# cocowy1/Cost-Volume-Aggregation-in-Stereo-Matching-Revisited

Hardware: AMD Instinct MI355X
Metric: cost-volumes/sec (fwd+bwd) at 544x960 D=192 (higher is better)
Workload: dtype f32

## Files before the change

cost-volume-aggregation-in-stereo-matching-revisited_amd/csrc/pointwise.hip:

```cpp
#include "bn_math.h"
#include "../../include/dca_hip.h"

__global__ __launch_bounds__(256) void bn_stats_kernel(const float* __restrict__ x, double* __restrict__ part, int N,
                                                       int C, long S, int nchunk, long chunk_len, int vec) {
  const int c = blockIdx.x, ch = blockIdx.y, tid = threadIdx.x;
  const long s0 = ch * chunk_len, s1 = min(S, s0 + chunk_len);
  const float K = x[(long)c * S];
  if (ch == 0 && tid == 0) part[(long)C * nchunk * 2 + c] = (double)K;
  float s = 0.f, ss = 0.f;
  for (int n = 0; n < N; ++n) {
    const float* p = x + ((long)n * C + c) * S;
    if (vec) {
      for (long i = s0 + 4 * tid; i < s1; i += 1024) {
        float4 v = *(const float4*)(p + i);
        v.x -= K; v.y -= K; v.z -= K; v.w -= K;
        s += (v.x + v.y) + (v.z + v.w);
        ss += (v.x * v.x + v.y * v.y) + (v.z * v.z + v.w * v.w);
      }
    } else {
      for (long i = s0 + tid; i < s1; i += 256) {
        const float v = p[i] - K;
        s += v;
        ss += v * v;
      }
// ... 590 lines not shown
  }
}

__global__ __launch_bounds__(256) void avgpool3d_fwd_tiled_kernel(const float* __restrict__ x, float* __restrict__ y,
                                                                  int Di, int Hi, int Wi, int Do, int Ho, int Wo) {
  constexpr int TH = 8, TW = 32, FH = 2 * TH + 1, PW = 2 * TW + 2;
  __shared__ __attribute__((aligned(16))) float tile[3 * FH * PW];
  const int tid = threadIdx.x, ow0 = blockIdx.x * TW, oh0 = blockIdx.y * TH;
  const int od = blockIdx.z % Do;
  const long nc = blockIdx.z / Do;
  const long plane = (long)Di * Hi * Wi;
  const __amdgpu_buffer_rsrc_t xr = dca_rsrc(x + nc * plane, plane * 4);
  constexpr int NQ = 3 * FH * 16, KQ = (NQ + 255) / 256;
  float4 rq[KQ];
#pragma unroll
  for (int k = 0; k < KQ; ++k) {
    const int it = tid + 256 * k, q = it & 15, row = it >> 4, a = row / FH, b = row - a * FH;
    const int d = 2 * od - 1 + a, h = 2 * oh0 - 1 + b, w = 2 * ow0 + 4 * q;
    const int ok = (int)(it < NQ) & (int)((unsigned)d < (unsigned)Di) & (int)((unsigned)h < (unsigned)Hi) & (int)(w < Wi);
    rq[k] = dca_bload4(xr, ((d * Hi + h) * Wi + w) * 4, ok);
  }
  float redge = 0.f;
  {
    const int a = tid / FH, b = tid - a * FH;
    const int d = 2 * od - 1 + a, h = 2 * oh0 - 1 + b, w = 2 * ow0 - 1;
    const int ok = (int)(tid < 3 * FH) & (int)((unsigned)d < (unsigned)Di) & (int)((unsigned)h < (unsigned)Hi) &
                   (int)((unsigned)w < (unsigned)Wi);
    redge = dca_bload1(xr, ((d * Hi + h) * Wi + w) * 4, ok);
  }
#pragma unroll
  for (int k = 0; k < KQ; ++k) {
    const int it = tid + 256 * k;
    if (it < NQ) {
      float* p = tile + (it >> 4) * PW + 1 + 4 * (it & 15);
      p[0] = rq[k].x; p[1] = rq[k].y; p[2] = rq[k].z; p[3] = rq[k].w;
    }
  }
  if (tid < 3 * FH) tile[tid * PW] = redge;
  __syncthreads();
  const int hl = tid >> 5, wl = tid & 31, oh = oh0 + hl, ow = ow0 + wl;
  if (oh >= Ho || ow >= Wo) return;
  float s = 0.f;
#pragma unroll
  for (int kd = 0; kd < 3; ++kd)
#pragma unroll
    for (int kh = 0; kh < 3; ++kh) {
      const float* row = tile + (kd * FH + 2 * hl + kh) * PW + 2 * wl;
      const float2 lo = *(const float2*)row;
      s += lo.x;
      s += lo.y;
      s += row[2];
    }
  y[((nc * Do + od) * Ho + oh) * (long)Wo + ow] = s * (1.0f / 27.0f);
}

__global__ __launch_bounds__(256) void avgpool3d_bwd_vec_kernel(const float* __restrict__ gy, float* __restrict__ gx,
                                                                const float* __restrict__ res, const float* __restrict__ res2,
                                                                int Di, int Hi, int Wi, int Do, int Ho, int Wo) {
  const int BD = Di / 2 + 1, BH = Hi / 2 + 1;
  const int bd = (int)(blockIdx.x % BD);
  const long nc = blockIdx.x / BD;
  const long plane = (long)Do * Ho * Wo;
  const __amdgpu_buffer_rsrc_t gr = dca_rsrc(gy + nc * plane, plane * 4);
  const int WQ = Wi >> 2, HQ = BH * WQ, end = min(HQ, ((int)blockIdx.y + 1) * 1024);
  for (int i = blockIdx.y * 1024 + threadIdx.x; i < end; i += 256) {
    const int bh = i / WQ, t = i - bh * WQ, c0 = 2 * t;
    float g[2][2][3];
#pragma unroll
    for (int a = 0; a < 2; ++a)
#pragma unroll
      for (int b = 0; b < 2; ++b)
#pragma unroll
        for (int c = 0; c < 3; ++c) {
          const int od = bd - 1 + a, oh = bh - 1 + b, ow = c0 + c;
          const int ok = (int)((unsigned)od < (unsigned)Do) & (int)((unsigned)oh < (unsigned)Ho) & (int)(ow < Wo);
          g[a][b][c] = dca_bload1(gr, ((od * Ho + oh) * Wo + ow) * 4, ok);
        }
#pragma unroll
    for (int pd = 0; pd < 2; ++pd) {
      const int d = 2 * bd - 1 + pd;
      if ((unsigned)d >= (unsigned)Di) continue;
#pragma unroll
      for (int ph = 0; ph < 2; ++ph) {
        const int h = 2 * bh - 1 + ph;
        if ((unsigned)h >= (unsigned)Hi) continue;
        float o[4];
#pragma unroll
        for (int e = 0; e < 4; ++e) {
          float s = 0.f;
#pragma unroll
          for (int a = pd; a < 2; ++a)
#pragma unroll
            for (int b = ph; b < 2; ++b) {
              s += g[a][b][e >> 1];
              s += (e & 1) ? g[a][b][(e + 1) >> 1] : 0.f;
            }
          o[e] = s * (1.0f / 27.0f);
        }
        const long off = ((nc * Di + d) * Hi + h) * (long)Wi + 4 * t;
        if (res) {
          const float4 r = *(const float4*)(res + off);
          o[0] += r.x; o[1] += r.y; o[2] += r.z; o[3] += r.w;
        }
        if (res2) {
          const float4 r = *(const float4*)(res2 + off);
          o[0] += r.x; o[1] += r.y; o[2] += r.z; o[3] += r.w;
// ... 72 lines not shown
        if (wh == 0.f) continue;
        const float* row = p + ((long)od * Ho + oh) * Wo;
        float r = 0.f;
        for (int ow = ow0; ow <= ow1; ++ow) r += lin_w(ow, w, rs, Wi) * row[ow];
        acc += wd * wh * r;
      }
    }
    gx[idx] = acc;
  }
}

__global__ __launch_bounds__(256) void trilinear_up2_fwd_kernel(const float* __restrict__ x, float* __restrict__ y,
                                                                int Di, int Hi, int Wi) {
  const int mw = blockIdx.x * 64 + (threadIdx.x & 63), mh = blockIdx.y * 4 + (threadIdx.x >> 6);
  const int md = blockIdx.z % Di;
  const long nc = blockIdx.z / Di;
  if (mw >= Wi || mh >= Hi) return;
  const float* p = x + nc * Di * Hi * Wi;
  const int dm = max(md - 1, 0), dp = min(md + 1, Di - 1), hm = max(mh - 1, 0), hp = min(mh + 1, Hi - 1);
  const int wm = max(mw - 1, 0), wp = min(mw + 1, Wi - 1);
  float r0[3][3], r1[3][3];
  const int ds[3] = {dm, md, dp}, hs[3] = {hm, mh, hp};
#pragma unroll
  for (int a = 0; a < 3; ++a)
#pragma unroll
    for (int b = 0; b < 3; ++b) {
      const float* row = p + ((long)ds[a] * Hi + hs[b]) * Wi;
      const float xm = row[wm], x0 = row[mw], xp = row[wp];
      r0[a][b] = 0.25f * xm + 0.75f * x0;
      r1[a][b] = 0.75f * x0 + 0.25f * xp;
    }
  const int Ho = 2 * Hi, Wo = 2 * Wi;
  float* q = y + nc * (2L * Di) * Ho * Wo;
#pragma unroll
  for (int pd = 0; pd < 2; ++pd)
#pragma unroll
    for (int ph = 0; ph < 2; ++ph) {
      const int a0 = pd ? 1 : 0, a1 = pd ? 2 : 1, b0 = ph ? 1 : 0, b1 = ph ? 2 : 1;
      const float wa0 = pd ? 0.75f : 0.25f, wa1 = pd ? 0.25f : 0.75f, wb0 = ph ? 0.75f : 0.25f, wb1 = ph ? 0.25f : 0.75f;
      float2 o;
      o.x = wa0 * (wb0 * r0[a0][b0] + wb1 * r0[a0][b1]) + wa1 * (wb0 * r0[a1][b0] + wb1 * r0[a1][b1]);
      o.y = wa0 * (wb0 * r1[a0][b0] + wb1 * r1[a0][b1]) + wa1 * (wb0 * r1[a1][b0] + wb1 * r1[a1][b1]);
      *(float2*)(q + ((long)(2 * md + pd) * Ho + 2 * mh + ph) * Wo + 2 * mw) = o;
    }
}

__device__ __forceinline__ void up2_bwd_w(int i, int n, float w[4]) {
  w[0] = (i > 0) ? 0.25f : 0.f;
  w[1] = (i > 0) ? 0.75f : 1.0f;
  w[2] = (i < n - 1) ? 0.75f : 1.0f;
  w[3] = (i < n - 1) ? 0.25f : 0.f;
}

__global__ __launch_bounds__(256) void trilinear_up2_bwd_kernel(const float* __restrict__ gy, float* __restrict__ gx,
                                                                int Di, int Hi, int Wi) {
  const int w = blockIdx.x * 256 + threadIdx.x, h = blockIdx.y;
  const int d = blockIdx.z % Di;
  const long nc = blockIdx.z / Di;
  const int Ho = 2 * Hi, Wo = 2 * Wi;
  const long plane = (2L * Di) * Ho * Wo;
  const __amdgpu_buffer_rsrc_t gr = dca_rsrc(gy + nc * plane, plane * 4);
  const int wok = (int)(w < Wi);
  float wd[4], wh[4], ww[4];
  up2_bwd_w(d, Di, wd); up2_bwd_w(h, Hi, wh); up2_bwd_w(w, Wi, ww);
  float acc = 0.f;
#pragma unroll
  for (int a = 0; a < 4; ++a) {
    const int od = 2 * d - 1 + a;
#pragma unroll
    for (int b = 0; b < 4; ++b) {
      const int oh = 2 * h - 1 + b;
      const int ok = wok & (int)(wd[a] != 0.f) & (int)(wh[b] != 0.f);
      const int off = ((od * Ho + oh) * Wo + 2 * w) * 4;
      const float2 mid = dca_bload2(gr, off, ok);
      const float lo = dca_bload1(gr, off - 4, ok & (int)(ww[0] != 0.f));
      const float hi = dca_bload1(gr, off + 8, ok & (int)(ww[3] != 0.f));
      float r = ww[1] * mid.x + ww[2] * mid.y;
      r += ww[0] * lo;
      r += ww[3] * hi;
      acc += wd[a] * wh[b] * r;
    }
  }
  if (wok) gx[((nc * Di + d) * Hi + h) * Wi + w] = acc;
}

__global__ __launch_bounds__(256) void trilinear_up2_bwd_tiled_kernel(const float* __restrict__ gy, float* __restrict__ gx,
                                                                      int Di, int Hi, int Wi) {
  constexpr int TH = 8, TW = 32, FH = 2 * TH + 2, FW = 2 * TW + 2, PW = FW + 2;
  __shared__ __attribute__((aligned(16))) float tile[4 * FH * PW];
  const int tid = threadIdx.x, w0 = blockIdx.x * TW, h0 = blockIdx.y * TH;
  const int d = blockIdx.z % Di;
  const long nc = blockIdx.z / Di;
  const int Do = 2 * Di, Ho = 2 * Hi, Wo = 2 * Wi;
  const long plane = (long)Do * Ho * Wo;
  const __amdgpu_buffer_rsrc_t gr = dca_rsrc(gy + nc * plane, plane * 4);
  constexpr int NQ = 4 * FH * 16, KQ = (NQ + 255) / 256;
  float4 rq[KQ];
#pragma unroll
  for (int k = 0; k < KQ; ++k) {
    const int it = tid + 256 * k, q = it & 15, row = it >> 4, a = row / FH, b = row - a * FH;
    const int od = 2 * d - 1 + a, oh = 2 * h0 - 1 + b, ow = 2 * w0 + 4 * q;
    const int ok = (int)(it < NQ) & (int)((unsigned)od < (unsigned)Do) & (int)((unsigned)oh < (unsigned)Ho) &
                   (int)(ow < Wo);
    rq[k] = dca_bload4(gr, ((od * Ho + oh) * Wo + ow) * 4, ok);
  }
  float redge = 0.f;
  {
    const int side = tid & 1, row = tid >> 1, a = row / FH, b = row - a * FH;
    const int od = 2 * d - 1 + a, oh = 2 * h0 - 1 + b, ow = side ? 2 * w0 + 2 * TW : 2 * w0 - 1;
    const int ok = (int)(tid < 4 * FH * 2) & (int)((unsigned)od < (unsigned)Do) & (int)((unsigned)oh < (unsigned)Ho) &
                   (int)((unsigned)ow < (unsigned)Wo);
    redge = dca_bload1(gr, ((od * Ho + oh) * Wo + ow) * 4, ok);
  }
#pragma unroll
  for (int k = 0; k < KQ; ++k) {
    const int it = tid + 256 * k;
    if (it < NQ) {
      float* p = tile + (it >> 4) * PW + 1 + 4 * (it & 15);
      p[0] = rq[k].x; p[1] = rq[k].y; p[2] = rq[k].z; p[3] = rq[k].w;
    }
  }
  if (tid < 4 * FH * 2) tile[(tid >> 1) * PW + ((tid & 1) ? FW - 1 : 0)] = redge;
  __syncthreads();
  const int hl = tid >> 5, wl = tid & 31, h = h0 + hl, w = w0 + wl;
  if (h >= Hi || w >= Wi) return;
  float wd[4], wh[4], ww[4];
  up2_bwd_w(d, Di, wd); up2_bwd_w(h, Hi, wh); up2_bwd_w(w, Wi, ww);
  float acc = 0.f;
#pragma unroll
  for (int a = 0; a < 4; ++a)
#pragma unroll
    for (int b = 0; b < 4; ++b) {
      const float* row = tile + (a * FH + 2 * hl + b) * PW + 2 * wl;
      const float2 lo = *(const float2*)row, hi = *(const float2*)(row + 2);
      float r = ww[1] * lo.y + ww[2] * hi.x;
      r += ww[0] * lo.x;
      r += ww[3] * hi.y;
      acc += wd[a] * wh[b] * r;
    }
  gx[((nc * Di + d) * Hi + h) * Wi + w] = acc;
}

static int ew_grid(long total) {
  long g = (total + 255) / 256;
  return (int)(g < 8192 ? (g > 0 ? g : 1) : 8192);
}

static void chunking(long S, int C, int* nchunk, long* chunk_len) {
  long want = (2048 + C - 1) / C;
  if (want > 256) want = 256;
  long len = (S + want - 1) / want;
  len = ((len + 1023) / 1024) * 1024;
  *chunk_len = len;
  *nchunk = (int)((S + len - 1) / len);
}

extern "C" int dca_bn_num_chunks(int C, long S) {
  int n; long l;
  chunking(S, C, &n, &l);
  return n;
}
extern "C" int dca_bn_pack_chunks(int C, long S) {
  int n; long l;
  chunking(S, (C + 7) / 8, &n, &l);
  return n;
}

extern "C" int dca_bn_stats(const float* x, double* part, int N, int C, long S, hipStream_t stream) {
  DCA_REQUIRE(x && part && N > 0 && C > 0 && S > 0 && C <= 65535);
  int nchunk; long len;
  chunking(S, C, &nchunk, &len);
  const int vec = (S % 4 == 0) && (((uintptr_t)x & 15) == 0);
  hipLaunchKernelGGL(bn_stats_kernel, dim3(C, nchunk), dim3(256), 0, stream, x, part, N, C, S, nchunk, len, vec);
  return dca_launch_status();
}

extern "C" int dca_bn_finalize(const double* part, int nchunk, double count, const float* gamma, const float* beta,
                               float* running_mean, float* running_var, float momentum, float eps, int training,
                               float* stats, int* zexps, const unsigned* rpre_slots, int rpre_n,
                               const unsigned* rpost_slots, int rpost_n, int C, hipStream_t stream) {
  DCA_REQUIRE(stats && C > 0 && (training ? (part != nullptr && nchunk > 0) : (running_mean && running_var)));
  DCA_REQUIRE(zexps == nullptr || training);
  DCA_REQUIRE((rpre_slots == nullptr || (rpre_n > 0 && rpre_n <= DCA_AMAX_CSLOTS)) &&
              (rpost_slots == nullptr || (rpost_n > 0 && rpost_n <= DCA_AMAX_CSLOTS)));
  hipLaunchKernelGGL(bn_finalize_kernel, dim3(C), dim3(64), 0, stream, part, nchunk, count, gamma, beta,
                     running_mean, running_var, momentum, eps, training, stats, zexps, rpre_slots, rpre_n, rpost_slots,
                     rpost_n, C);
  return dca_launch_status();
}

extern "C" int dca_bn_finalize_centered(const double* part, int nchunk, const float* gamma, const float* beta,
                                        float* running_mean, float* running_var, float momentum, float eps, float* stats,
                                        int* zexps, const unsigned* rpre_slots, int rpre_n, const unsigned* rpost_slots,
// ... 107 lines not shown
  hipLaunchKernelGGL(bn_bwd_finalize_kernel, dim3(C), dim3(64), 0, stream, part, nchunk, count, dgb, C, stats, training,
                     (const unsigned*)nullptr, (const unsigned*)nullptr, 0, (int*)nullptr);
  hipLaunchKernelGGL(bn_bwd_finalize_kernel, dim3(C), dim3(64), 0, stream, (const double*)part_r, nchunk, count, dgb_r, C,
                     stats_r, training, (const unsigned*)nullptr, (const unsigned*)nullptr, 0, (int*)nullptr);
  hipLaunchKernelGGL(bn_bwd_apply_kernel, dim3(nchunk, C), dim3(256), 0, stream, dz, y, (const float*)nullptr, stats, dgb, dy,
                     g_out, N, C, S, len, slope, training, vec, dmax, y_r, stats_r);
  return dca_launch_status();
}

extern "C" int dca_bn_backward_reduce(const float* dz, const float* y, const float* stats, double* part, float* dgb, int N,
                                      int C, long S, float slope, int training, hipStream_t stream) {
  DCA_REQUIRE(dz && y && stats && part && dgb && N > 0 && C > 0 && S > 0 && C <= 65535);
  int nchunk; long len;
  chunking(S, C, &nchunk, &len);
  const int vec = (S % 4 == 0) && ((((uintptr_t)dz | (uintptr_t)y) & 15) == 0);
  hipLaunchKernelGGL(bn_bwd_reduce_kernel, dim3(C, nchunk), dim3(256), 0, stream, dz, y, (const float*)nullptr, stats, part,
                     N, C, S, nchunk, len, slope, vec, (unsigned*)nullptr, (const float*)nullptr, (const float*)nullptr,
                     (double*)nullptr);
  hipLaunchKernelGGL(bn_bwd_finalize_kernel, dim3(C), dim3(64), 0, stream, part, nchunk, (double)N * (double)S, dgb, C,
                     stats, training, (const unsigned*)nullptr, (const unsigned*)nullptr, 0, (int*)nullptr);
  return dca_launch_status();
}

void dca_internal_bn_chunking(long S, int C, int* nchunk, long* chunk_len) { chunking(S, C, nchunk, chunk_len); }

int dca_internal_bn_bwd_finalize(const double* part, int nchunk, double count, float* dgb, int C, const float* stats,
                                 int training, const unsigned* gmax, const unsigned* ymax, int ymax_slots, int* dyexps,
                                 hipStream_t stream) {
  hipLaunchKernelGGL(bn_bwd_finalize_kernel, dim3(C), dim3(64), 0, stream, part, nchunk, count, dgb, C, stats, training, gmax,
                     ymax, ymax_slots, dyexps);
  return dca_launch_status();
}

extern "C" int dca_bn_backward_pack(const float* dz, const float* y, const float* stats, double* part, float* dgb, void* dyp,
                                    int* dyexps, unsigned* gmax, const unsigned* ymax, int ymax_slots, int N, int C, long S,
                                    float slope, int training, hipStream_t stream) {
  DCA_REQUIRE(dz && y && stats && part && dgb && dyp && dyexps && gmax && N > 0 && C > 0 && C % 8 == 0 && S > 0 && C <= 65535);
  DCA_REQUIRE((ymax == nullptr || (ymax_slots > 0 && ymax_slots <= DCA_AMAX_CSLOTS)) && ((((uintptr_t)dyp) & 15) == 0));
  int nchunk; long len;
  chunking(S, C, &nchunk, &len);
  const uintptr_t al = (uintptr_t)dz | (uintptr_t)y;
  const int vec = (S % 4 == 0) && ((al & 15) == 0);
  hipLaunchKernelGGL(bn_bwd_reduce_kernel, dim3(C, nchunk), dim3(256), 0, stream, dz, y, (const float*)nullptr, stats, part,
                     N, C, S, nchunk, len, slope, vec, gmax, (const float*)nullptr, (const float*)nullptr, (double*)nullptr);
  hipLaunchKernelGGL(bn_bwd_finalize_kernel, dim3(C), dim3(64), 0, stream, part, nchunk, (double)N * (double)S, dgb, C,
                     stats, training, (const unsigned*)gmax, ymax, ymax_slots, dyexps);
  int pchunk; long plen;
  chunking(S, C / 8, &pchunk, &plen);
  hipLaunchKernelGGL(bn_bwd_apply_pack_kernel, dim3(pchunk, C / 8), dim3(256), 0, stream, dz, y, stats, dgb, dyexps,
                     (char*)dyp, N, C, S, plen, slope, training);
  return dca_launch_status();
}

extern "C" int dca_avgpool3d_fwd(const float* x, float* y, long NC, int Di, int Hi, int Wi, hipStream_t stream) {
  DCA_REQUIRE(x && y && NC > 0 && Di > 0 && Hi > 0 && Wi > 0);
  const int Do = (Di + 1) / 2, Ho = (Hi + 1) / 2, Wo = (Wi + 1) / 2;
  DCA_REQUIRE((long)Di * Hi * Wi * 4 < 0x7ffffff0L && NC * Do < 0x7fffffffL);
  if (Wi % 4 == 0 && (((uintptr_t)x) & 15) == 0 && NC * Do <= 65535 && cdiv(Ho, 8) <= 65535) {
    hipLaunchKernelGGL(avgpool3d_fwd_tiled_kernel, dim3(cdiv(Wo, 32), cdiv(Ho, 8), (unsigned)(NC * Do)), dim3(256), 0, stream,
                       x, y, Di, Hi, Wi, Do, Ho, Wo);
    return dca_launch_status();
  }
  hipLaunchKernelGGL(avgpool3d_fwd_kernel, dim3((unsigned)(NC * Do), cdiv((long)Ho * Wo, 1024)), dim3(256), 0, stream, x,
                     y, Di, Hi, Wi, Do, Ho, Wo);
  return dca_launch_status();
}

extern "C" int dca_avgpool3d_bwd(const float* gy, float* gx, const float* res, const float* res2, long NC, int Di, int Hi,
                                 int Wi, hipStream_t stream) {
  DCA_REQUIRE(gy && gx && NC > 0 && Di > 0 && Hi > 0 && Wi > 0 && (res || !res2));
  const int Do = (Di + 1) / 2, Ho = (Hi + 1) / 2, Wo = (Wi + 1) / 2;
  DCA_REQUIRE((long)Di * Hi * Wi * 4 < 0x7ffffff0L && NC * Di < 0x7fffffffL);
  if (Wi % 4 == 0 && ((((uintptr_t)gx) | ((uintptr_t)res) | ((uintptr_t)res2)) & 15) == 0) {
    hipLaunchKernelGGL(avgpool3d_bwd_vec_kernel, dim3((unsigned)(NC * (Di / 2 + 1)), cdiv((long)(Hi / 2 + 1) * (Wi / 4), 1024)),
                       dim3(256), 0, stream, gy, gx, res, res2, Di, Hi, Wi, Do, Ho, Wo);
    return dca_launch_status();
  }
  hipLaunchKernelGGL(avgpool3d_bwd_kernel, dim3((unsigned)(NC * Di), cdiv((long)Hi * Wi, 1024)), dim3(256), 0, stream, gy,
                     gx, res, res2, Di, Hi, Wi, Do, Ho, Wo);
  return dca_launch_status();
}

extern "C" int dca_trilinear_fwd(const float* x, float* y, long NC, int Di, int Hi, int Wi, int scale,
                                 hipStream_t stream) {
  DCA_REQUIRE(x && y && NC > 0 && Di > 0 && Hi > 0 && Wi > 0 && scale >= 1);
  if (scale == 2 && Hi <= 65535 && NC * Di <= 65535 && (((uintptr_t)y & 7) == 0)) {
    hipLaunchKernelGGL(trilinear_up2_fwd_kernel, dim3(cdiv(Wi, 64), cdiv(Hi, 4), (unsigned)(NC * Di)), dim3(256), 0, stream,
                       x, y, Di, Hi, Wi);
    return dca_launch_status();
  }
  const long total = NC * Di * Hi * Wi * scale * scale * scale;
  hipLaunchKernelGGL(trilinear_fwd_kernel, dim3(ew_grid(total)), dim3(256), 0, stream, x, y, NC, Di, Hi, Wi, scale);
  return dca_launch_status();
}

extern "C" int dca_trilinear_bwd(const float* gy, float* gx, long NC, int Di, int Hi, int Wi, int scale,
                                 hipStream_t stream) {
  DCA_REQUIRE(gy && gx && NC > 0 && Di > 0 && Hi > 0 && Wi > 0 && scale >= 1);
  if (scale == 2 && cdiv(Hi, 8) <= 65535 && NC * Di <= 65535 && 32L * Di * Hi * Wi < 0x7ffffff0L && Wi % 2 == 0 &&
      (((uintptr_t)gy & 15) == 0)) {
    hipLaunchKernelGGL(trilinear_up2_bwd_tiled_kernel, dim3(cdiv(Wi, 32), cdiv(Hi, 8), (unsigned)(NC * Di)), dim3(256), 0,
                       stream, gy, gx, Di, Hi, Wi);
    return dca_launch_status();
  }
  if (scale == 2 && Hi <= 65535 && NC * Di <= 65535 && 32L * Di * Hi * Wi < 0x7ffffff0L && (((uintptr_t)gy & 7) == 0)) {
    hipLaunchKernelGGL(trilinear_up2_bwd_kernel, dim3(cdiv(Wi, 256), Hi, (unsigned)(NC * Di)), dim3(256), 0, stream, gy, gx,
                       Di, Hi, Wi);
    return dca_launch_status();
  }
  hipLaunchKernelGGL(trilinear_bwd_kernel, dim3(ew_grid(NC * Di * Hi * Wi)), dim3(256), 0, stream, gy, gx, NC, Di, Hi,
                     Wi, scale);
  return dca_launch_status();
}
```

cost-volume-aggregation-in-stereo-matching-revisited_amd/ops.py:

```python
from __future__ import annotations

import ctypes
import os
import threading

import torch

from ._call import _C, _L, _chk, _ptr, _raw_device, _raw_stream, _req, _req_no_grad, _stream, _vp
from .guided import GUIDE, guide_params, hints_to_quarter


def _opt(t, name):
    return None if t is None else _req(t, name)


class _GwcVolume(torch.autograd.Function):
    @staticmethod
    def forward(ctx, ref, tgt, maxdisp, num_groups):
        ref, tgt = _req(ref, "build_gwc_volume"), _req(tgt, "build_gwc_volume")
        B, C, H, W = ref.shape
        vol = torch.empty((B, num_groups, maxdisp, H, W), device=ref.device, dtype=torch.float32)
        with torch.cuda.device_of(ref):
            _chk(_L().dca_gwc_volume_fwd(_ptr(ref), _ptr(tgt), _ptr(vol), B, C, H, W, maxdisp, num_groups, _stream()),
                 "dca_gwc_volume_fwd")
# ... 242 lines not shown
        _chk(_L().dca_softargmin_stats(_ptr(x), _ptr(out), B, K, HW, min(radius, K), _stream()), "dca_softargmin_stats")
    return out


class _UpSoftArgmin(torch.autograd.Function):

    @staticmethod
    def forward(ctx, logits, scale):
        logits = _req(logits, "up_softargmin")
        B, n, hc, wc = logits.shape
        disp = torch.empty((B, 1, scale * hc, scale * wc), device=logits.device, dtype=torch.float32)
        with torch.cuda.device_of(logits):
            _chk(_L().dca_up_softargmin_fwd(_ptr(logits), _ptr(disp), B, n, hc, wc, scale, _stream()),
                 "dca_up_softargmin_fwd")
        ctx.save_for_backward(logits)
        ctx.scale = scale
        return disp

    @staticmethod
    def backward(ctx, g):
        (logits,) = ctx.saved_tensors
        g = _req(g, "up_softargmin.backward")
        B, n, hc, wc = logits.shape
        s = ctx.scale
        g1 = torch.empty((B, n, s * hc, s * wc), device=logits.device, dtype=torch.float32)
        gl = torch.empty_like(logits)
        with torch.cuda.device_of(logits):
            _chk(_L().dca_up_softargmin_bwd(_ptr(logits), _ptr(g), _ptr(g1), _ptr(gl), B, n, hc, wc, s, _stream()),
                 "dca_up_softargmin_bwd")
        return gl, None


def up_softargmin(logits, scale):
    if logits.shape[1] > 64 or logits.shape[1] < 2 or scale not in (2, 4, 8):
        return softargmin(trilinear_upsample(logits.unsqueeze(1), scale).squeeze(1))
    return _UpSoftArgmin.apply(logits, int(scale))


def _round_up(a, m):
    return (a + m - 1) // m * m


_CONV_MODE = os.environ.get("DCA_CONV", "x2")
CONV_X3 = _CONV_MODE != "fp32"
CONV_X2 = _CONV_MODE == "x2"
WGRAD_S2_X2 = os.environ.get("DCA_WGRAD_S2", "x2") != "fp32"
DECONV_X3 = os.environ.get("DCA_DECONV", "x3") != "fp32"
C1_WGRAD_FUSED = os.environ.get("DCA_C1_WGRAD", "fused") != "expand"
CONV_S2_X2 = os.environ.get("DCA_CONV_S2", "x2") != "fp32"
BN_FUSE = os.environ.get("DCA_BN_FUSE", "1") != "0"
C1_BWD_FUSE = os.environ.get("DCA_C1_BWD", "fused") != "split"
SKIP_FOLD = os.environ.get("DCA_SKIP_FOLD", "1") != "0"
C1_HEAD_BWD = os.environ.get("DCA_C1_HEAD_BWD", "fused") != "split"
_X3_MIN_WORKGROUPS = 1


AMAX_STATS = {"tagged": 0, "computed": 0, "packed": 0}
CSLOTS = _C["DCA_AMAX_CSLOTS"]
AMAX_EMIT = os.environ.get("DCA_AMAX_EMIT", "1") != "0"
PACK = os.environ.get("DCA_PACK", "1") != "0"


def _cslots(C, device):
    if not AMAX_EMIT:
        return None
    return torch.empty((C * CSLOTS,), device=device, dtype=torch.int32)


def _ver(t):
    return None if t.is_inference() else t._version


def _tag_cmax(t, slots, nslots):
    if slots is not None:
        t._dca_cmax = (slots, int(nslots), _ver(t))
    return t


def _tag_px2(t, exps):
    t._dca_px2 = (exps,)
    return t


def _tag_exps(t, exps):
    t._dca_exps = (exps, _ver(t))


def _tag_twin(t, twin):
    t._dca_twin = (twin, _ver(t))


def _tag_ok(t, name):
    tag = getattr(t, name, None)
    if tag is not None and tag[-1] == _ver(t) and tag[0].device == t.device:
        return tag
    return None


def _copy_tags(src, dst):
    cmax, exps, twin = _tag_ok(src, "_dca_cmax"), _tag_ok(src, "_dca_exps"), _tag_ok(src, "_dca_twin")
    if cmax is not None:
        _tag_cmax(dst, cmax[0], cmax[1])
    if exps is not None:
        _tag_exps(dst, exps[0])
    if twin is not None:
        _tag_twin(dst, twin[0])
# ... 1016 lines not shown
def convbn3d(x, conv, bn, slope=1.0, res_pre=None, res_post=None, x2=None, alias=False, pack_out=False):
    transposed = isinstance(conv, torch.nn.ConvTranspose3d)
    stride = conv.stride[0]
    if isinstance(res_pre, _SkipBn):
        if pack_out != "both" or alias:
            raise RuntimeError("convbn3d: a folded skip branch needs pack_out='both' (convbn3d_pair, skip_into)")
        if BN_FUSE and conv.weight.shape[0 if not transposed else 1] > 1:
            y, part = _Conv3d.apply(x, x2, conv.weight, int(stride), bool(transposed), True)
        else:
            y, part = conv3d(x, conv.weight, stride, transposed, x2), None
        return bn_skip_act(y, bn, slope, res_pre, res_post, part if (part is not None and part.numel()) else None)
    if alias:
        fuse = (PAIR_FUSE and torch.is_grad_enabled() and x.requires_grad and _k3s1(conv.weight, stride, transposed, x2)
                and _lp_dtype() is None and x.dtype == torch.float32)
        if not fuse:
            return convbn3d(x, conv, bn, slope, res_pre, res_post, x2), x
        stats = bool(BN_FUSE and bn.training)
        pdy = _pack_dy_ok(x, None, conv, False, 1, res_pre)
        out = _Conv3d.apply(x, None, conv.weight, 1, False, stats, True, pdy)
        y, part, xa = (out[0], out[1], out[2]) if stats else (out[0], None, out[1])
        z = bn_act(y, bn, slope, res_pre, res_post, part if (part is not None and part.numel()) else None,
                   pack_out=pack_out, pack_dy=pdy)
        return z, xa
    if not bn.training and not torch.is_grad_enabled():
        lp = _lp_dtype()
        if lp is not None and not transposed and stride == 1 and conv.kernel_size[0] == 3 and x2 is None:
            with torch.cuda.device_of(x):
                stats = bn_eval_affine(bn)
            C = bn.num_features
            return conv3d_lp(x, conv.weight, lp, stats[2 * C:3 * C], stats[3 * C:], slope, res_pre, res_post,
                             out_dtype=x.dtype)
        xx = _req(x, "convbn3d")
        with torch.cuda.device_of(xx):
            stats = bn_eval_affine(bn)
        C = bn.num_features
        return conv3d_fused_inference(xx, conv.weight, stride, transposed, stats[2 * C:3 * C], stats[3 * C:], slope,
                                      res_pre, res_post, x2)
    if BN_FUSE and bn.training and conv.weight.shape[0 if not transposed else 1] > 1 and _lp_dtype() is None:
        pdy = _pack_dy_ok(x, x2, conv, transposed, stride, res_pre)
        lazy = not transposed and _c1_bwd_route(x, x2, conv.weight, res_pre) == "fused"
        y, part = _Conv3d.apply(x, x2, conv.weight, int(stride), bool(transposed), True, False, pdy, lazy)
        return bn_act(y, bn, slope, res_pre, res_post, part if part.numel() else None, pack_out=pack_out, pack_dy=pdy,
                      lazy_dy=lazy)
    if not transposed and _lp_dtype() is None and _c1_bwd_route(x, x2, conv.weight, res_pre) == "fused":
        y = _Conv3d.apply(x, x2, conv.weight, int(stride), False, False, False, False, True)
        return bn_act(y, bn, slope, res_pre, res_post, lazy_dy=True)
    if _is_packed(x) and _pack_dy_ok(x, x2, conv, transposed, stride, res_pre):
        y = _Conv3d.apply(x, x2, conv.weight, int(stride), bool(transposed), False, False, True)
        return bn_act(y, bn, slope, res_pre, res_post, pack_dy=True)
    y = conv3d(x, conv.weight, stride, transposed, x2)
    return bn_act(y, bn, slope, res_pre, res_post)


class _AvgPool3d(torch.autograd.Function):
    @staticmethod
    def forward(ctx, x):
        x = _req(x, "avg_pool3d")
        N, C, D, H, W = x.shape
        y = torch.empty((N, C, (D + 1) // 2, (H + 1) // 2, (W + 1) // 2), device=x.device, dtype=torch.float32)
        with torch.cuda.device_of(x):
            _chk(_L().dca_avgpool3d_fwd(_ptr(x), _ptr(y), N * C, D, H, W, _stream()), "dca_avgpool3d_fwd")
        ctx.shape = tuple(x.shape)
        return y

    @staticmethod
    def backward(ctx, gy):
        gy = _req(gy, "avg_pool3d.backward")
        N, C, D, H, W = ctx.shape
        gx = torch.empty(ctx.shape, device=gy.device, dtype=torch.float32)
        with torch.cuda.device_of(gy):
            _chk(_L().dca_avgpool3d_bwd(_ptr(gy), _ptr(gx), None, None, N * C, D, H, W, _stream()), "dca_avgpool3d_bwd")
        return gx


class _PoolFork(torch.autograd.Function):

    @staticmethod
    def forward(ctx, x, third):
        x = _req(x, "avg_pool3d")
        N, C, D, H, W = x.shape
        y = torch.empty((N, C, (D + 1) // 2, (H + 1) // 2, (W + 1) // 2), device=x.device, dtype=torch.float32)
        with torch.cuda.device_of(x):
            _chk(_L().dca_avgpool3d_fwd(_ptr(x), _ptr(y), N * C, D, H, W, _stream()), "dca_avgpool3d_fwd")
        ctx.shape = tuple(x.shape)
        ctx.set_materialize_grads(False)
        if third:
            return y, x.view_as(x), x.view_as(x)
        return y, x.view_as(x)

    @staticmethod
    def backward(ctx, gy, gx2, gx3=None):
        extra = [g for g in (gx2, gx3) if g is not None]
        if gy is None:
            return (extra[0] + extra[1] if len(extra) == 2 else (extra[0] if extra else None)), None
        gy = _req(gy, "avg_pool3d.backward")
        res = _opt(extra[0], "avg_pool3d.backward") if extra else None
        res2 = _opt(extra[1], "avg_pool3d.backward") if len(extra) == 2 else None
        N, C, D, H, W = ctx.shape
        gx = torch.empty(ctx.shape, device=gy.device, dtype=torch.float32)
        with torch.cuda.device_of(gy):
            _chk(_L().dca_avgpool3d_bwd(_ptr(gy), _ptr(gx), _ptr(res), _ptr(res2), N * C, D, H, W, _stream()),
                 "dca_avgpool3d_bwd")
        return gx, None


def avg_pool3d_fork(x, third=False):
    if PAIR_FUSE and torch.is_grad_enabled() and x.requires_grad and x.dtype == torch.float32:
        outs = _PoolFork.apply(x, bool(third))
        for o in outs[1:]:
            _copy_tags(x, o)
        return outs
    return (avg_pool3d_k3s2p1(x), x, x) if third else (avg_pool3d_k3s2p1(x), x)


class _Trilinear(torch.autograd.Function):
    @staticmethod
    def forward(ctx, x, scale):
        x = _req(x, "interpolate")
        N, C, D, H, W = x.shape
        y = torch.empty((N, C, D * scale, H * scale, W * scale), device=x.device, dtype=torch.float32)
        with torch.cuda.device_of(x):
            _chk(_L().dca_trilinear_fwd(_ptr(x), _ptr(y), N * C, D, H, W, scale, _stream()), "dca_trilinear_fwd")
        ctx.meta = (tuple(x.shape), scale)
        return y

    @staticmethod
    def backward(ctx, gy):
        shape, scale = ctx.meta
        gy = _req(gy, "interpolate.backward")
        N, C, D, H, W = shape
        gx = torch.empty(shape, device=gy.device, dtype=torch.float32)
        with torch.cuda.device_of(gy):
            _chk(_L().dca_trilinear_bwd(_ptr(gy), _ptr(gx), N * C, D, H, W, scale, _stream()), "dca_trilinear_bwd")
        return gx, None


def avg_pool3d_k3s2p1(x):
    return _AvgPool3d.apply(x)


def trilinear_upsample(x, scale):
    return _Trilinear.apply(x, int(scale))


class _ContextInject(torch.autograd.Function):
    @staticmethod
    def forward(ctx, x, preds):
        x, preds = _req(x, "context_inject"), _req(preds, "context_inject.preds")
        B, C, n = x.shape[:3]
        HW = x.shape[3] * x.shape[4]
        key = torch.empty_like(x)
        kstar = torch.empty((B, HW), device=x.device, dtype=torch.int32)
        e = torch.empty((B, HW), device=x.device, dtype=torch.float32)
        pm = torch.empty_like(e)
        denom = torch.empty((B, n), device=x.device, dtype=torch.float32)
        part = torch.empty((B * ((HW + 255) // 256) * n,), device=x.device, dtype=torch.float32)
        with torch.cuda.device_of(x):
            _chk(_L().dca_context_inject_fwd(_ptr(x), _ptr(preds), _ptr(key), _ptr(kstar), _ptr(e), _ptr(pm),
                                             _ptr(denom), _ptr(part), B, C, n, HW, _stream()), "dca_context_inject_fwd")
        ctx.save_for_backward(x, preds, kstar, e, pm, denom)
        ctx.mark_non_differentiable(kstar)
        return key, kstar

    @staticmethod
    def backward(ctx, dkey, _unused):
        x, preds, kstar, e, pm, denom = ctx.saved_tensors
        dkey = _req(dkey, "context_inject.backward")
        B, C, n = x.shape[:3]
        HW = x.shape[3] * x.shape[4]
        dx, dpreds = torch.empty_like(x), torch.empty_like(preds)
        dw = torch.empty_like(e)
        T = torch.empty_like(denom)
        part = torch.empty((B * ((HW + 255) // 256) * n,), device=x.device, dtype=torch.float32)
        with torch.cuda.device_of(x):
            _chk(_L().dca_context_inject_bwd(_ptr(dkey), _ptr(x), _ptr(preds), _ptr(kstar), _ptr(e), _ptr(pm),
                                             _ptr(denom), _ptr(dx), _ptr(dpreds), _ptr(dw), _ptr(T), _ptr(part), B, C,
                                             n, HW, _stream()), "dca_context_inject_bwd")
        return dx, dpreds


class _DispAttention(torch.autograd.Function):
    @staticmethod
    def forward(ctx, q, k, v):
        q, k, v = _req(q, "attention.q"), _req(k, "attention.k"), _req(v, "attention.v")
        B, C, n = q.shape[:3]
        HW = q.shape[3] * q.shape[4]
# ... 328 lines not shown
```

include/dca_hip.h:

```cpp
#ifndef DCA_HIP_H
#define DCA_HIP_H

#include <hip/hip_runtime_api.h>

#ifdef __cplusplus
extern "C" {
#endif

#define DCA_ABI_VERSION 21
int dca_abi_version(void);

#define DCA_BF16 1
#define DCA_FP16 2

int dca_gwc_volume_fwd(const float* ref, const float* tgt, float* vol, int B, int C, int H, int W, int maxdisp,
                       int num_groups, hipStream_t stream);
int dca_gwc_volume_bwd(const float* gvol, const float* ref, const float* tgt, float* gref, float* gtgt, int B, int C,
                       int H, int W, int maxdisp, int num_groups, hipStream_t stream);
long dca_gwc_volume_bwd_rows(int B, int C, int H, int W, int maxdisp, int num_groups);
int dca_concat_volume_fwd(const float* ref, const float* tgt, float* vol, int B, int C, int H, int W, int maxdisp,
                          hipStream_t stream);
int dca_concat_volume_bwd(const float* gvol, float* gref, float* gtgt, int B, int C, int H, int W, int maxdisp,
                          hipStream_t stream);

// ... 81 lines not shown
long dca_conv3d_s2x2_weight_bytes(int Cin, int Cout);
int dca_conv3d_s2x2_prep_weight(const float* w, void* wx, int A, int B, int src_ab, int flip, const unsigned* x_slots,
                                int nslots, int* xexps, hipStream_t stream);
long dca_conv3d_s2x2_out_slots(int N, int Cout, int Di, int Hi, int Wi);
int dca_conv3d_s2x2_forward(const float* x, const int* xexps, const void* wx, float* y, const float* scale, const float* shift,
                            float slope, const float* res_post, unsigned* y_cmax, int N, int Cin, int Cout, int Di, int Hi, int Wi,
                            hipStream_t stream);
long dca_conv3d_wgrad_x2_workspace(int N, int Cx, int Cy, int D, int H, int W);
int dca_conv3d_wgrad_x2(const void* x, int x_packed, const int* xexps, const void* dy, int dy_packed, const int* yexps,
                        float* part, float* dw, int N, int Cx, int Cy, int D, int H, int W, long s_cy, long s_cx,
                        hipStream_t stream);

int dca_conv3d_c1_gather(const float* T, float* y, int N, int D, int H, int W, hipStream_t stream);
int dca_conv3d_c1_wgrad(const float* x, const float* dy, float* part, float* dw, int N, int C, int D, int H, int W,
                        hipStream_t stream);
int dca_conv3d_c1_expand(const float* dy, float* G, int N, int D, int H, int W, hipStream_t stream);
int dca_conv3d_c1_bwd_data(const float* dy, const float* w, float* dx, int N, int C, int D, int H, int W,
                           hipStream_t stream);

int dca_bn_num_chunks(int C, long S);
int dca_bn_pack_chunks(int C, long S);
int dca_bn_stats(const float* x, double* part, int N, int C, long S, hipStream_t stream);
int dca_bn_finalize(const double* part, int nchunk, double count, const float* gamma, const float* beta,
                    float* running_mean, float* running_var, float momentum, float eps, int training, float* stats,
                    int* zexps, const unsigned* rpre_slots, int rpre_n, const unsigned* rpost_slots, int rpost_n, int C,
                    hipStream_t stream);
int dca_bn_apply(const float* y, const float* stats, const float* res_pre, const float* res_post, float* z, int N,
                 int C, long S, float slope, unsigned* zmax, unsigned* ymax, hipStream_t stream);
int dca_bn_apply_pack(const float* y, const float* stats, const int* zexps, void* zp, int N, int C, long S, float slope,
                      unsigned* ymax, const float* res_pre, const float* res_post, float* zf, unsigned* zmax,
                      hipStream_t stream);
int dca_bn_backward(const float* dz, const float* y, const float* res_pre, const float* stats, double* part,
                    float* dgb, float* dy, float* g_out, int N, int C, long S, float slope, int training,
                    unsigned* dmax, hipStream_t stream);
int dca_bn_backward_reduce(const float* dz, const float* y, const float* stats, double* part, float* dgb, int N, int C,
                           long S, float slope, int training, hipStream_t stream);
int dca_bn_backward_pack(const float* dz, const float* y, const float* stats, double* part, float* dgb, void* dyp,
                         int* dyexps, unsigned* gmax, const unsigned* ymax, int ymax_slots, int N, int C, long S,
                         float slope, int training, hipStream_t stream);
int dca_bn_backward_pack_c1_chunks(int N, int D, int H, int W);
int dca_bn_backward_pack_c1_grid(int N, int D, int H, int W);
int dca_bn_backward_pack_c1(const float* dlogit, const float* w_head, const float* y, const float* stats, double* part,
                            float* dgb, void* dyp, int* dyexps, unsigned* gmax, const unsigned* ymax, int ymax_slots, int N,
                            int C, int D, int H, int W, float slope, int training, hipStream_t stream);
int dca_bn_skip_max(const float* y_r, const float* stats_r, int N, int C, long S, unsigned* slots, hipStream_t stream);
int dca_bn_apply_pack_skip(const float* y, const float* stats, const int* zexps, void* zp, int N, int C, long S, float slope,
                           unsigned* ymax, const float* y_r, const float* stats_r, const float* res_post, float* zf,
                           unsigned* zmax, hipStream_t stream);
int dca_bn_backward_skip(const float* dz, const float* y, const float* y_r, const float* stats, const float* stats_r,
                         double* part, double* part_r, float* dgb, float* dgb_r, float* dy, float* g_out, int N, int C,
                         long S, float slope, int training, unsigned* dmax, hipStream_t stream);

int dca_avgpool3d_fwd(const float* x, float* y, long NC, int Di, int Hi, int Wi, hipStream_t stream);
int dca_avgpool3d_bwd(const float* gy, float* gx, const float* res, const float* res2, long NC, int Di, int Hi, int Wi,
                     hipStream_t stream);

int dca_trilinear_fwd(const float* x, float* y, long NC, int Di, int Hi, int Wi, int scale, hipStream_t stream);
int dca_trilinear_bwd(const float* gy, float* gx, long NC, int Di, int Hi, int Wi, int scale, hipStream_t stream);

int dca_context_inject_fwd(const float* x, const float* preds, float* key, int* kstar, float* e, float* pm,
                           float* denom, float* part, int B, int C, int n, long HW, hipStream_t stream);
int dca_context_inject_bwd(const float* dkey, const float* x, const float* preds, const int* kstar, const float* e,
                           const float* pm, const float* denom, float* dx, float* dpreds, float* dw, float* T,
                           float* part, int B, int C, int n, long HW, hipStream_t stream);

int dca_disp_attention_fwd(const float* q, const float* k, const float* v, float* out, int B, int C, int n, long HW,
                           hipStream_t stream);
int dca_disp_attention_bwd(const float* q, const float* k, const float* v, const float* dout, float* dq, float* dk,
                           float* dv, int B, int C, int n, long HW, hipStream_t stream);

int dca_convex_up4_fwd(const float* mask_logits, const float* disp, float* up, int B, int h, int w, hipStream_t stream);
int dca_convex_up4_bwd(const float* mask_logits, const float* disp, const float* gup, float* glogits, float* gdisp,
                       float* wk, int B, int h, int w, hipStream_t stream);

long dca_focal_loss_workspace(int nlev, int B, long HW);
int dca_focal_loss_fwd(const float* const* ests, const float* weights, int nlev, const float* gt, double* work,
                       float* out, int B, int K, long HW, float focal_coefficient, hipStream_t stream);
int dca_focal_loss_bwd(const float* const* ests, float* const* gests, const float* weights, int nlev, const float* gt,
                       const double* work, const float* gloss, int B, int K, long HW, float focal_coefficient,
                       hipStream_t stream);

long dca_conv3d_lp_weight_bytes(int Cin, int Cout);
int dca_conv3d_lp_prep_weight(const float* w, void* wx, int A, int B, int src_ab, int flip, int dtype,
                              hipStream_t stream);
int dca_conv3d_lp_forward(const void* x, const void* wx, void* y, const float* scale, const float* shift,
                          const void* res_pre, const void* res_post, float slope, int N, int Cin, int Cout, int D, int H,
                          int W, int dtype, int in_f32, int out_f32, hipStream_t stream);

long dca_conv1_lp_weight_bytes(int C1, int C2);
int dca_conv1_lp_prep_weight(const float* w, void* wfrag, int Cout, int C1, int C2, int dtype, hipStream_t stream);
int dca_conv1_lp_forward(const void* x, const void* x2, const void* wfrag, void* y, const float* scale,
                         const float* shift, const void* res_pre, const void* res_post, float slope, int N, int C1,
                         int C2, int Cout, long S, int dtype, int out_f32, hipStream_t stream);

int dca_conv3d_forward_mixed(const void* x, const float* wt, void* y, const float* scale, const float* shift,
                             const void* res_pre, const void* res_post, float slope, int N, int Cin, int Cout, int CinPad,
                             int Di, int Hi, int Wi, int Do, int Ho, int Wo, int transposed, int dtype,
                             hipStream_t stream);
long dca_conv3d_s2_lp_weight_bytes(int Cin);
int dca_conv3d_s2_lp_prep_weight(const float* w, void* wx, int Cin, int Cout, int dtype, hipStream_t stream);
int dca_conv3d_s2_lp_forward(const void* x, const void* wx, float* y, const float* scale, const float* shift, float slope,
                             int N, int Cin, int Cout, int D, int H, int W, int dtype, hipStream_t stream);
int dca_deconv3d_lp_forward(const float* x, const void* wx, void* y, const float* scale, const float* shift,
                            const void* res_pre, const void* res_post, float slope, int N, int Cin, int Cout, int Di,
                            int Hi, int Wi, int dtype, hipStream_t stream);
int dca_avgpool3d_lp_fwd(const void* x, float* y, long NC, int Di, int Hi, int Wi, int dtype, hipStream_t stream);
int dca_trilinear_up2_lp_fwd(const float* x, void* y, long NC, int Di, int Hi, int Wi, int dtype, hipStream_t stream);

#define DCA_EVAL_REC 8
long dca_disp_metrics_workspace(int B, int H, int W);
int dca_disp_metrics(const float* pred, const float* gt, const unsigned char* mask, double* rec, void* workspace, int B,
// ... 181 lines not shown
```

Before: 43.53.

## March avgpool fwd and trilinear-up2 bwd along depth with rolling LDS tiles

Adds depth-marching variants of the avgpool3d forward and trilinear up2 backward kernels. Each block walks a segment of output depth slices and keeps a rolling ring of input planes in shared memory, so overlapping depth halo planes are loaded once instead of re-fetched by every per-slice block. The next plane pair is prefetched into registers while the current slice is computed. This cuts redundant global reads of the 3x and 4x depth stencils, at the cost of fewer blocks (segments sized to about 8192 columns) and two barriers per slice. The marching path is the default, and the old tiled path stays selectable through an env var.

```diff
diff --git a/cost-volume-aggregation-in-stereo-matching-revisited_amd/csrc/pointwise.hip b/cost-volume-aggregation-in-stereo-matching-revisited_amd/csrc/pointwise.hip
--- a/cost-volume-aggregation-in-stereo-matching-revisited_amd/csrc/pointwise.hip
+++ b/cost-volume-aggregation-in-stereo-matching-revisited_amd/csrc/pointwise.hip
@@ -666,6 +666,78 @@
       s += row[2];
     }
   y[((nc * Do + od) * Ho + oh) * (long)Wo + ow] = s * (1.0f / 27.0f);
+}
+
+__global__ __launch_bounds__(256) void avgpool3d_fwd_march_kernel(const float* __restrict__ x, float* __restrict__ y,
+                                                                  int Di, int Hi, int Wi, int Do, int Ho, int Wo,
+                                                                  int seg_len, int nseg) {
+  constexpr int TH = 8, TW = 32, FH = 2 * TH + 1, PW = 2 * TW + 2;
+  __shared__ __attribute__((aligned(16))) float tile[3 * FH * PW];
+  const int tid = threadIdx.x, ow0 = blockIdx.x * TW, oh0 = blockIdx.y * TH;
+  const int seg = blockIdx.z % nseg;
+  const long nc = blockIdx.z / nseg;
+  const int obeg = seg * seg_len, oend = min(Do, obeg + seg_len);
+  const long plane = (long)Di * Hi * Wi;
+  const __amdgpu_buffer_rsrc_t xr = dca_rsrc(x + nc * plane, plane * 4);
+  constexpr int NQ = 2 * FH * 16, KQ = (NQ + 255) / 256, NE = 2 * FH;
+  float4 rq[KQ];
+  float redge;
+  auto load_pair = [&](int p0, int amin) {
+#pragma unroll
+    for (int k = 0; k < KQ; ++k) {
+      const int it = tid + 256 * k, q = it & 15, row = it >> 4, a = row / FH, b = row - a * FH;
+      const int d = p0 + a, h = 2 * oh0 - 1 + b, w = 2 * ow0 + 4 * q;
+      const int ok = (int)(it < NQ) & (int)(a >= amin) & (int)((unsigned)d < (unsigned)Di) &
+                     (int)((unsigned)h < (unsigned)Hi) & (int)(w < Wi);
+      rq[k] = dca_bload4(xr, ((d * Hi + h) * Wi + w) * 4, ok);
+    }
+    const int a = tid / FH, b = tid - a * FH;
+    const int d = p0 + a, h = 2 * oh0 - 1 + b, w = 2 * ow0 - 1;
+    const int ok = (int)(tid < NE) & (int)(a >= amin) & (int)((unsigned)d < (unsigned)Di) &
+                   (int)((unsigned)h < (unsigned)Hi) & (int)((unsigned)w < (unsigned)Wi);
+    redge = dca_bload1(xr, ((d * Hi + h) * Wi + w) * 4, ok);
+  };
+  auto store_pair = [&](int slot0, int slot1, int amin) {
+#pragma unroll
+    for (int k = 0; k < KQ; ++k) {
+      const int it = tid + 256 * k, row = it >> 4, a = row / FH, b = row - a * FH;
+      if (it < NQ && a >= amin) {
+        float* p = tile + ((a ? slot1 : slot0) * FH + b) * PW + 1 + 4 * (it & 15);
+        p[0] = rq[k].x; p[1] = rq[k].y; p[2] = rq[k].z; p[3] = rq[k].w;
+      }
+    }
+    const int a = tid / FH, b = tid - a * FH;
+    if (tid < NE && a >= amin) tile[((a ? slot1 : slot0) * FH + b) * PW] = redge;
+  };
+  const int hl = tid >> 5, wl = tid & 31, oh = oh0 + hl, ow = ow0 + wl;
+  const bool live = oh < Ho && ow < Wo;
+  int sl = 0;
+  load_pair(2 * obeg - 2, 1);
+  store_pair(0, sl, 1);
+  load_pair(2 * obeg, 0);
+  for (int od = obeg; od < oend; ++od) {
+    const int s1 = sl == 2 ? 0 : sl + 1, s2 = s1 == 2 ? 0 : s1 + 1;
+    store_pair(s1, s2, 0);
+    __syncthreads();
+    if (od + 1 < oend) load_pair(2 * od + 2, 0);
+    if (live) {
+      const int slot[3] = {sl, s1, s2};
+      float s = 0.f;
+#pragma unroll
+      for (int kd = 0; kd < 3; ++kd)
+#pragma unroll
+        for (int kh = 0; kh < 3; ++kh) {
+          const float* row = tile + (slot[kd] * FH + 2 * hl + kh) * PW + 2 * wl;
+          const float2 lo = *(const float2*)row;
+          s += lo.x;
+          s += lo.y;
+          s += row[2];
+        }
+      y[((nc * Do + od) * Ho + oh) * (long)Wo + ow] = s * (1.0f / 27.0f);
+    }
+    __syncthreads();
+    sl = s2;
+  }
 }
 
 __global__ __launch_bounds__(256) void avgpool3d_bwd_vec_kernel(const float* __restrict__ gy, float* __restrict__ gx,
@@ -844,6 +916,26 @@
   w[3] = (i < n - 1) ? 0.25f : 0.f;
 }
 
+template <int A, int B>
+__device__ __forceinline__ float up2_bwd_term(float acc, float wd, float wh, const float ww[4], float x0, float x1, float x2,
+                                              float x3) {
+  float r = (B == 3 && A >= 1) ? __fmaf_rn(ww[2], x2, __fmul_rn(ww[1], x1)) : __fmaf_rn(ww[1], x1, __fmul_rn(ww[2], x2));
+  r = __fmaf_rn(ww[0], x0, r);
+  r = __fmaf_rn(ww[3], x3, r);
+  return __fmaf_rn(__fmul_rn(wd, wh), r, acc);
+}
+template <int A = 0, int B = 0, class RowOf>
+__device__ __forceinline__ float up2_bwd_sum(float acc, const float wd[4], const float wh[4], const float ww[4], RowOf row_of) {
+  if constexpr (A == 4) {
+    return acc;
+  } else {
+    const float* row = row_of(A, B);
+    const float2 lo = *(const float2*)row, hi = *(const float2*)(row + 2);
+    acc = up2_bwd_term<A, B>(acc, wd[A], wh[B], ww, lo.x, lo.y, hi.x, hi.y);
+    return up2_bwd_sum<(B == 3 ? A + 1 : A), (B == 3 ? 0 : B + 1)>(acc, wd, wh, ww, row_of);
+  }
+}
+
 __global__ __launch_bounds__(256) void trilinear_up2_bwd_kernel(const float* __restrict__ gy, float* __restrict__ gx,
                                                                 int Di, int Hi, int Wi) {
   const int w = blockIdx.x * 256 + threadIdx.x, h = blockIdx.y;
@@ -918,19 +1010,72 @@
   if (h >= Hi || w >= Wi) return;
   float wd[4], wh[4], ww[4];
   up2_bwd_w(d, Di, wd); up2_bwd_w(h, Hi, wh); up2_bwd_w(w, Wi, ww);
-  float acc = 0.f;
-#pragma unroll
-  for (int a = 0; a < 4; ++a)
-#pragma unroll
-    for (int b = 0; b < 4; ++b) {
-      const float* row = tile + (a * FH + 2 * hl + b) * PW + 2 * wl;
-      const float2 lo = *(const float2*)row, hi = *(const float2*)(row + 2);
-      float r = ww[1] * lo.y + ww[2] * hi.x;
-      r += ww[0] * lo.x;
-      r += ww[3] * hi.y;
-      acc += wd[a] * wh[b] * r;
-    }
+  const float acc = up2_bwd_sum(0.f, wd, wh, ww, [&](int a, int b) { return tile + (a * FH + 2 * hl + b) * PW + 2 * wl; });
   gx[((nc * Di + d) * Hi + h) * Wi + w] = acc;
+}
+
+__global__ __launch_bounds__(256) void trilinear_up2_bwd_march_kernel(const float* __restrict__ gy, float* __restrict__ gx,
+                                                                      int Di, int Hi, int Wi, int seg_len, int nseg) {
+  constexpr int TH = 8, TW = 32, FH = 2 * TH + 2, FW = 2 * TW + 2, PW = FW + 2;
+  __shared__ __attribute__((aligned(16))) float tile[4 * FH * PW];
+  const int tid = threadIdx.x, w0 = blockIdx.x * TW, h0 = blockIdx.y * TH;
+  const int seg = blockIdx.z % nseg;
+  const long nc = blockIdx.z / nseg;
+  const int dbeg = seg * seg_len, dend = min(Di, dbeg + seg_len);
+  const int Do = 2 * Di, Ho = 2 * Hi, Wo = 2 * Wi;
+  const long plane = (long)Do * Ho * Wo;
+  const __amdgpu_buffer_rsrc_t gr = dca_rsrc(gy + nc * plane, plane * 4);
+  constexpr int NQ = 2 * FH * 16, KQ = (NQ + 255) / 256, NE = 2 * FH * 2;
+  float4 rq[KQ];
+  float redge;
+  auto load_pair = [&](int p0) {
+#pragma unroll
+    for (int k = 0; k < KQ; ++k) {
+      const int it = tid + 256 * k, q = it & 15, row = it >> 4, a = row / FH, b = row - a * FH;
+      const int od = p0 + a, oh = 2 * h0 - 1 + b, ow = 2 * w0 + 4 * q;
+      const int ok = (int)(it < NQ) & (int)((unsigned)od < (unsigned)Do) & (int)((unsigned)oh < (unsigned)Ho) &
+                     (int)(ow < Wo);
+      rq[k] = dca_bload4(gr, ((od * Ho + oh) * Wo + ow) * 4, ok);
+    }
+    const int side = tid & 1, row = tid >> 1, a = row / FH, b = row - a * FH;
+    const int od = p0 + a, oh = 2 * h0 - 1 + b, ow = side ? 2 * w0 + 2 * TW : 2 * w0 - 1;
+    const int ok = (int)(tid < NE) & (int)((unsigned)od < (unsigned)Do) & (int)((unsigned)oh < (unsigned)Ho) &
+                   (int)((unsigned)ow < (unsigned)Wo);
+    redge = dca_bload1(gr, ((od * Ho + oh) * Wo + ow) * 4, ok);
+  };
+  auto store_pair = [&](int p0) {
+    float* base = tile + ((p0 + 1) & 3) * (FH * PW);
+#pragma unroll
+    for (int k = 0; k < KQ; ++k) {
+      const int it = tid + 256 * k;
+      if (it < NQ) {
+        float* p = base + (it >> 4) * PW + 1 + 4 * (it & 15);
+        p[0] = rq[k].x; p[1] = rq[k].y; p[2] = rq[k].z; p[3] = rq[k].w;
+      }
+    }
+    if (tid < NE) base[(tid >> 1) * PW + ((tid & 1) ? FW - 1 : 0)] = redge;
+  };
+  const int hl = tid >> 5, wl = tid & 31, h = h0 + hl, w = w0 + wl;
+  const bool live = h < Hi && w < Wi;
+  float wh[4], ww[4];
+  up2_bwd_w(h, Hi, wh); up2_bwd_w(w, Wi, ww);
+  load_pair(2 * dbeg - 1);
+  store_pair(2 * dbeg - 1);
+  load_pair(2 * dbeg + 1);
+  for (int d = dbeg; d < dend; ++d) {
+    store_pair(2 * d + 1);
+    __syncthreads();
+    if (d + 1 < dend) load_pair(2 * d + 3);
+    if (live) {
+      float wd[4];
+      up2_bwd_w(d, Di, wd);
+      const float acc = up2_bwd_sum(0.f, wd, wh, ww, [&](int a, int b) {
+        return tile + (((2 * d + a) & 3) * FH + 2 * hl + b) * PW + 2 * wl;
+      });
+      gx[((nc * Di + d) * Hi + h) * Wi + w] = acc;
+    }
+    __syncthreads();
+  }
 }
 
 static int ew_grid(long total) {
@@ -1144,11 +1289,30 @@
   return dca_launch_status();
 }
 
-extern "C" int dca_avgpool3d_fwd(const float* x, float* y, long NC, int Di, int Hi, int Wi, hipStream_t stream) {
+static int glue_march_seg(long NC, int Dc, int Hc, int Wc) {
+  const long cols = NC * cdiv(Hc, 8) * cdiv(Wc, 32);
+  long nseg = (8192 + cols - 1) / cols;
+  const long most = cdiv(Dc, 8);
+  nseg = nseg < most ? nseg : most;
+  return cdiv(Dc, nseg);
+}
+
+extern "C" long dca_glue_march_seg(long NC, int Dc, int Hc, int Wc) {
+  if (NC <= 0 || Dc <= 0 || Hc <= 0 || Wc <= 0) return -1;
+  return glue_march_seg(NC, Dc, Hc, Wc);
+}
+
+static int avgpool3d_fwd_launch(const float* x, float* y, long NC, int Di, int Hi, int Wi, bool march, hipStream_t stream) {
   DCA_REQUIRE(x && y && NC > 0 && Di > 0 && Hi > 0 && Wi > 0);
   const int Do = (Di + 1) / 2, Ho = (Hi + 1) / 2, Wo = (Wi + 1) / 2;
   DCA_REQUIRE((long)Di * Hi * Wi * 4 < 0x7ffffff0L && NC * Do < 0x7fffffffL);
   if (Wi % 4 == 0 && (((uintptr_t)x) & 15) == 0 && NC * Do <= 65535 && cdiv(Ho, 8) <= 65535) {
+    if (march) {
+      const int len = glue_march_seg(NC, Do, Ho, Wo), nseg = cdiv(Do, len);
+      hipLaunchKernelGGL(avgpool3d_fwd_march_kernel, dim3(cdiv(Wo, 32), cdiv(Ho, 8), (unsigned)(NC * nseg)), dim3(256), 0,
+                         stream, x, y, Di, Hi, Wi, Do, Ho, Wo, len, nseg);
+      return dca_launch_status();
+    }
     hipLaunchKernelGGL(avgpool3d_fwd_tiled_kernel, dim3(cdiv(Wo, 32), cdiv(Ho, 8), (unsigned)(NC * Do)), dim3(256), 0, stream,
                        x, y, Di, Hi, Wi, Do, Ho, Wo);
     return dca_launch_status();
@@ -1156,6 +1320,13 @@
   hipLaunchKernelGGL(avgpool3d_fwd_kernel, dim3((unsigned)(NC * Do), cdiv((long)Ho * Wo, 1024)), dim3(256), 0, stream, x,
                      y, Di, Hi, Wi, Do, Ho, Wo);
   return dca_launch_status();
+}
+
+extern "C" int dca_avgpool3d_fwd(const float* x, float* y, long NC, int Di, int Hi, int Wi, hipStream_t stream) {
+  return avgpool3d_fwd_launch(x, y, NC, Di, Hi, Wi, true, stream);
+}
+extern "C" int dca_avgpool3d_fwd_tiled(const float* x, float* y, long NC, int Di, int Hi, int Wi, hipStream_t stream) {
+  return avgpool3d_fwd_launch(x, y, NC, Di, Hi, Wi, false, stream);
 }
 
 extern "C" int dca_avgpool3d_bwd(const float* gy, float* gx, const float* res, const float* res2, long NC, int Di, int Hi,
@@ -1186,11 +1357,17 @@
   return dca_launch_status();
 }
 
-extern "C" int dca_trilinear_bwd(const float* gy, float* gx, long NC, int Di, int Hi, int Wi, int scale,
-                                 hipStream_t stream) {
+static int trilinear_bwd_launch(const float* gy, float* gx, long NC, int Di, int Hi, int Wi, int scale, bool march,
+                                hipStream_t stream) {
   DCA_REQUIRE(gy && gx && NC > 0 && Di > 0 && Hi > 0 && Wi > 0 && scale >= 1);
   if (scale == 2 && cdiv(Hi, 8) <= 65535 && NC * Di <= 65535 && 32L * Di * Hi * Wi < 0x7ffffff0L && Wi % 2 == 0 &&
       (((uintptr_t)gy & 15) == 0)) {
+    if (march) {
+      const int len = glue_march_seg(NC, Di, Hi, Wi), nseg = cdiv(Di, len);
+      hipLaunchKernelGGL(trilinear_up2_bwd_march_kernel, dim3(cdiv(Wi, 32), cdiv(Hi, 8), (unsigned)(NC * nseg)), dim3(256), 0,
+                         stream, gy, gx, Di, Hi, Wi, len, nseg);
+      return dca_launch_status();
+    }
     hipLaunchKernelGGL(trilinear_up2_bwd_tiled_kernel, dim3(cdiv(Wi, 32), cdiv(Hi, 8), (unsigned)(NC * Di)), dim3(256), 0,
                        stream, gy, gx, Di, Hi, Wi);
     return dca_launch_status();
@@ -1204,3 +1381,12 @@
                      Wi, scale);
   return dca_launch_status();
 }
+
+extern "C" int dca_trilinear_bwd(const float* gy, float* gx, long NC, int Di, int Hi, int Wi, int scale,
+                                 hipStream_t stream) {
+  return trilinear_bwd_launch(gy, gx, NC, Di, Hi, Wi, scale, true, stream);
+}
+extern "C" int dca_trilinear_bwd_tiled(const float* gy, float* gx, long NC, int Di, int Hi, int Wi, int scale,
+                                       hipStream_t stream) {
+  return trilinear_bwd_launch(gy, gx, NC, Di, Hi, Wi, scale, false, stream);
+}
diff --git a/cost-volume-aggregation-in-stereo-matching-revisited_amd/ops.py b/cost-volume-aggregation-in-stereo-matching-revisited_amd/ops.py
--- a/cost-volume-aggregation-in-stereo-matching-revisited_amd/ops.py
+++ b/cost-volume-aggregation-in-stereo-matching-revisited_amd/ops.py
@@ -318,6 +318,7 @@
 C1_BWD_FUSE = os.environ.get("DCA_C1_BWD", "fused") != "split"
 SKIP_FOLD = os.environ.get("DCA_SKIP_FOLD", "1") != "0"
 C1_HEAD_BWD = os.environ.get("DCA_C1_HEAD_BWD", "fused") != "split"
+GLUE_TILED = os.environ.get("DCA_GLUE", "march") == "tiled"
 _X3_MIN_WORKGROUPS = 1
 
 
@@ -1440,6 +1441,14 @@
     return bn_act(y, bn, slope, res_pre, res_post)
 
 
+def _pool_fwd(x, y):
+    N, C, D, H, W = x.shape
+    if GLUE_TILED:
+        _chk(_L().dca_avgpool3d_fwd_tiled(_ptr(x), _ptr(y), N * C, D, H, W, _stream()), "dca_avgpool3d_fwd_tiled")
+    else:
+        _chk(_L().dca_avgpool3d_fwd(_ptr(x), _ptr(y), N * C, D, H, W, _stream()), "dca_avgpool3d_fwd")
+
+
 class _AvgPool3d(torch.autograd.Function):
     @staticmethod
     def forward(ctx, x):
@@ -1447,7 +1456,7 @@
         N, C, D, H, W = x.shape
         y = torch.empty((N, C, (D + 1) // 2, (H + 1) // 2, (W + 1) // 2), device=x.device, dtype=torch.float32)
         with torch.cuda.device_of(x):
-            _chk(_L().dca_avgpool3d_fwd(_ptr(x), _ptr(y), N * C, D, H, W, _stream()), "dca_avgpool3d_fwd")
+            _pool_fwd(x, y)
         ctx.shape = tuple(x.shape)
         return y
 
@@ -1469,7 +1478,7 @@
         N, C, D, H, W = x.shape
         y = torch.empty((N, C, (D + 1) // 2, (H + 1) // 2, (W + 1) // 2), device=x.device, dtype=torch.float32)
         with torch.cuda.device_of(x):
-            _chk(_L().dca_avgpool3d_fwd(_ptr(x), _ptr(y), N * C, D, H, W, _stream()), "dca_avgpool3d_fwd")
+            _pool_fwd(x, y)
         ctx.shape = tuple(x.shape)
         ctx.set_materialize_grads(False)
         if third:
@@ -1519,7 +1528,11 @@
         N, C, D, H, W = shape
         gx = torch.empty(shape, device=gy.device, dtype=torch.float32)
         with torch.cuda.device_of(gy):
-            _chk(_L().dca_trilinear_bwd(_ptr(gy), _ptr(gx), N * C, D, H, W, scale, _stream()), "dca_trilinear_bwd")
+            if GLUE_TILED:
+                _chk(_L().dca_trilinear_bwd_tiled(_ptr(gy), _ptr(gx), N * C, D, H, W, scale, _stream()),
+                     "dca_trilinear_bwd_tiled")
+            else:
+                _chk(_L().dca_trilinear_bwd(_ptr(gy), _ptr(gx), N * C, D, H, W, scale, _stream()), "dca_trilinear_bwd")
         return gx, None
 
 
diff --git a/include/dca_hip.h b/include/dca_hip.h
--- a/include/dca_hip.h
+++ b/include/dca_hip.h
@@ -157,11 +157,14 @@
                          long S, float slope, int training, unsigned* dmax, hipStream_t stream);
 
 int dca_avgpool3d_fwd(const float* x, float* y, long NC, int Di, int Hi, int Wi, hipStream_t stream);
+int dca_avgpool3d_fwd_tiled(const float* x, float* y, long NC, int Di, int Hi, int Wi, hipStream_t stream);
+long dca_glue_march_seg(long NC, int Dc, int Hc, int Wc);
 int dca_avgpool3d_bwd(const float* gy, float* gx, const float* res, const float* res2, long NC, int Di, int Hi, int Wi,
                      hipStream_t stream);
 
 int dca_trilinear_fwd(const float* x, float* y, long NC, int Di, int Hi, int Wi, int scale, hipStream_t stream);
 int dca_trilinear_bwd(const float* gy, float* gx, long NC, int Di, int Hi, int Wi, int scale, hipStream_t stream);
+int dca_trilinear_bwd_tiled(const float* gy, float* gx, long NC, int Di, int Hi, int Wi, int scale, hipStream_t stream);
 
 int dca_context_inject_fwd(const float* x, const float* preds, float* key, int* kstar, float* e, float* pm,
                            float* denom, float* part, int B, int C, int n, long HW, hipStream_t stream);
```

After: 43.83, median of 6. About the same (+0.7%).
